# LeoQLi/DeepSIR

Hardware: AMD Instinct MI355X
Metric: registered pairs/sec (5k-pt 3DMatch-shaped synthetic pairs, 5 registration iterations, KNN pyramid included) (higher is better)
Workload: dtype f32 (GEMMs as fp16-pair MFMA, fp32 accumulate; index decisions exact fp32)

## Files before the change

### deepsir_amd/csrc/agg_chain_h.hip

```cpp
#include <hip/hip_fp16.h>

#include "kernels.h"
#include "device_utils.h"

namespace dsir {

namespace {

typedef _Float16 h8 __attribute__((ext_vector_type(8)));

constexpr int SRS = 80;
constexpr int LDT = 68;

__device__ __forceinline__ void split8(const float4 u, const float4 v, h8& h, h8& l) {
  const float f[8] = {u.x, u.y, u.z, u.w, v.x, v.y, v.z, v.w};
#pragma unroll
  for (int k = 0; k < 8; ++k) {
    const _Float16 t = (_Float16)f[k];
    h[k] = t;
    l[k] = (_Float16)(f[k] - (float)t);
  }
}

#define DSIR_MFMA16(acc, a, b) acc = __builtin_amdgcn_mfma_f32_16x16x32_f16(a, b, acc, 0, 0, 0)

template <int RT>
__global__ __launch_bounds__(256, 2) void agg_chain_h_kernel(const AggArgs p) {
  __shared__ _Float16 Bs[2][2][64 * SRS];
  __shared__ float Ts[4][RT][16 * LDT];

  const int tid = threadIdx.x, lane = tid & 63, w = __builtin_amdgcn_readfirstlane(tid >> 6);
  const int fr = lane & 15, fq = lane >> 4;
  const int cloud = blockIdx.y;
  const int r0 = blockIdx.x * (64 * RT) + 16 * RT * w;

  auto chunk_src = [&](int i, int& layer, int& ld, int& col0, int& k0, int& nk) {
    if (i == 0) { layer = 0; ld = 32; col0 = 0; k0 = 0; nk = 32; }
    else if (i <= 2) { layer = 1; ld = 64; col0 = 64 * (i - 1); k0 = 0; nk = 64; }
    else if (i == 15) { layer = 4; ld = 64; col0 = 0; k0 = 0; nk = 64; }
    else {
      const int j = (i - 3) / 3, u = (i - 3) % 3;
      if (u < 2) { layer = 2; ld = 128; col0 = 64 * j; k0 = 64 * u; nk = 64; }
      else { layer = 3; ld = 256; col0 = 0; k0 = 64 * j; nk = 64; }
    }
  };
  h8 rwh[2][2], rwl[2][2];
  auto gload = [&](int i) {
    int layer, ld, col0, k0, nk;
    chunk_src(i, layer, ld, col0, k0, nk);
    const _Float16* Wh = reinterpret_cast<const _Float16*>(p.Wh[layer]);
    const _Float16* Wl = reinterpret_cast<const _Float16*>(p.Wl[layer]);
#pragma unroll
    for (int u = 0; u < 2; ++u) {
      const int f = tid + 256 * u;
      const int piece = min(f & 7, nk / 8 - 1);
      const int64_t o = (int64_t)(col0 + (f >> 3)) * ld + k0 + 8 * piece;
      rwh[i & 1][u] = *reinterpret_cast<const h8*>(Wh + o);
      rwl[i & 1][u] = *reinterpret_cast<const h8*>(Wl + o);
    }
  };
  auto lstore = [&](int buf, int i) {
#pragma unroll
    for (int u = 0; u < 2; ++u) {
      const int f = tid + 256 * u;
      *reinterpret_cast<h8*>(&Bs[buf][0][(f >> 3) * SRS + 8 * (f & 7)]) = rwh[i & 1][u];
      *reinterpret_cast<h8*>(&Bs[buf][1][(f >> 3) * SRS + 8 * (f & 7)]) = rwl[i & 1][u];
    }
  };
  int buf = 0, ci = 0;
  auto next_chunk = [&]() {
    if (ci + 1 < 16) lstore(buf ^ 1, ci + 1);
    __syncthreads();
    buf ^= 1;
    ++ci;
    if (ci + 2 < 16) gload(ci + 2);
  };

  gload(0);
  lstore(0, 0);
  gload(1);
  gload(2);

  {
    float w1[2], b1[2];
#pragma unroll
    for (int t = 0; t < 2; ++t) { w1[t] = p.W1[(16 * t + fr) * 4 + fq]; b1[t] = p.b1[16 * t + fr]; }
#pragma unroll
    for (int rt = 0; rt < RT; ++rt) {
      const int row = min(r0 + 16 * rt + fr, p.n - 1);
      const float a = fq < 3 ? p.xyz[cloud * p.xyz_cs + (int64_t)row * 3 + fq] : p.score[(int64_t)cloud * p.n + row];
      float* T = Ts[w][rt];
#pragma unroll
      for (int t = 0; t < 2; ++t) {
        f32x4 c = __builtin_amdgcn_mfma_f32_16x16x4f32(a, w1[t], f32x4{0.f, 0.f, 0.f, 0.f}, 0, 0, 0);
#pragma unroll
        for (int r = 0; r < 4; ++r) {
          float v = c[r] + b1[t];
          v = v < 0.f ? v * 0.2f : v;
          T[(4 * fq + r) * LDT + 16 * t + fr] = v;
        }
      }
    }
  }
  __syncthreads();

  struct AFrag { h8 h[2], l[2]; };
  auto spill = [&](float* T, const f32x4 (&acc)[4], const float* bias, bool act) {
    __builtin_amdgcn_wave_barrier();
#pragma unroll
    for (int t = 0; t < 4; ++t) {
      const float b = bias[16 * t + fr];
#pragma unroll
      for (int r = 0; r < 4; ++r) {
        float v = acc[t][r] + b;
        if (act) v = v < 0.f ? v * 0.2f : v;
        T[(4 * fq + r) * LDT + 16 * t + fr] = v;
      }
    }
    __builtin_amdgcn_wave_barrier();
  };
  auto read_frag = [&](const float* T, AFrag& a, bool both) {
    const float4* q = reinterpret_cast<const float4*>(T + fr * LDT + 8 * fq);
    split8(q[0], q[1], a.h[0], a.l[0]);
    if (both) split8(q[8], q[9], a.h[1], a.l[1]);
  };
  auto zero = [&](f32x4 (&acc)[RT][4]) {
#pragma unroll
    for (int rt = 0; rt < RT; ++rt)
#pragma unroll
      for (int t = 0; t < 4; ++t) acc[rt][t] = f32x4{0.f, 0.f, 0.f, 0.f};
  };
  auto mma = [&](f32x4 (&acc)[RT][4], const AFrag (&a)[RT], const int KS) {
    const _Float16* bh = &Bs[buf][0][fr * SRS + 8 * fq];
    const _Float16* bl = &Bs[buf][1][fr * SRS + 8 * fq];
#pragma unroll
    for (int t = 0; t < 4; ++t) {
#pragma unroll
      for (int s = 0; s < 2; ++s) {
        if (s < KS) {
          const h8 vh = *reinterpret_cast<const h8*>(bh + 16 * t * SRS + 32 * s);
          const h8 vl = *reinterpret_cast<const h8*>(bl + 16 * t * SRS + 32 * s);
#pragma unroll
          for (int rt = 0; rt < RT; ++rt) {
            DSIR_MFMA16(acc[rt][t], a[rt].l[s], vh);
            DSIR_MFMA16(acc[rt][t], a[rt].h[s], vl);
            DSIR_MFMA16(acc[rt][t], a[rt].h[s], vh);
          }
        }
      }
    }
  };

  AFrag a3[RT];
  {
    AFrag a2[RT];
#pragma unroll
    for (int rt = 0; rt < RT; ++rt) read_frag(Ts[w][rt], a2[rt], false);
    f32x4 acc[RT][4];
    zero(acc);
    mma(acc, a2, 1);
#pragma unroll
    for (int rt = 0; rt < RT; ++rt) {
      spill(Ts[w][rt], acc[rt], p.b2, true);
      read_frag(Ts[w][rt], a3[rt], true);
    }
    next_chunk();
  }

  AFrag a4[2][RT];
#pragma unroll
  for (int c = 0; c < 2; ++c) {
    f32x4 acc[RT][4];
    zero(acc);
    mma(acc, a3, 2);
#pragma unroll
    for (int rt = 0; rt < RT; ++rt) {
      spill(Ts[w][rt], acc[rt], p.b3 + 64 * c, true);
      read_frag(Ts[w][rt], a4[c][rt], true);
    }
    next_chunk();
  }

  f32x4 acc5[RT][4];
  zero(acc5);
  float fpre[RT][4][4];
#pragma unroll
  for (int j = 0; j < 4; ++j) {
    f32x4 acc[RT][4];
    zero(acc);
    if (j == 3) {
#pragma unroll
      for (int rt = 0; rt < RT; ++rt)
#pragma unroll
        for (int r = 0; r < 4; ++r) {
          const int row = min(r0 + 16 * rt + 4 * fq + r, p.n - 1);
          const float* f = p.F + ((int64_t)cloud * p.n + row) * 64 + fr;
#pragma unroll
          for (int t = 0; t < 4; ++t) fpre[rt][r][t] = f[16 * t];
        }
    }
    mma(acc, a4[0], 2);
    next_chunk();
    mma(acc, a4[1], 2);
    AFrag a5[RT];
#pragma unroll
    for (int rt = 0; rt < RT; ++rt) {
      spill(Ts[w][rt], acc[rt], p.b4 + 64 * j, true);
      read_frag(Ts[w][rt], a5[rt], true);
    }
    next_chunk();
    mma(acc5, a5, 2);
    next_chunk();
  }

  {
    AFrag a6[RT];
#pragma unroll
    for (int rt = 0; rt < RT; ++rt) {
      float* T = Ts[w][rt];
      __builtin_amdgcn_wave_barrier();
#pragma unroll
      for (int r = 0; r < 4; ++r) {
#pragma unroll
        for (int t = 0; t < 4; ++t) T[(4 * fq + r) * LDT + 16 * t + fr] = (acc5[rt][t][r] + p.b5[16 * t + fr]) + fpre[rt][r][t];
      }
      __builtin_amdgcn_wave_barrier();
      read_frag(T, a6[rt], true);
    }
    f32x4 acc[RT][4];
    zero(acc);
    mma(acc, a6, 2);
    float bv[4];
#pragma unroll
    for (int t = 0; t < 4; ++t) bv[t] = p.b6[16 * t + fr];
    float* Y = p.desc + (int64_t)cloud * p.n * 64;
#pragma unroll
    for (int rt = 0; rt < RT; ++rt) {
      float ss[4] = {0.f, 0.f, 0.f, 0.f};
      float v[4][4];
#pragma unroll
      for (int t = 0; t < 4; ++t)
#pragma unroll
        for (int r = 0; r < 4; ++r) {
          v[t][r] = acc[rt][t][r] + bv[t];
          ss[r] += v[t][r] * v[t][r];
        }
      const bool extras = p.sq || p.hi || p.packed_init;
      float* T = Ts[w][rt];
      if (extras) __builtin_amdgcn_wave_barrier();
#pragma unroll
      for (int r = 0; r < 4; ++r) {
        ss[r] += __shfl_xor(ss[r], 1); ss[r] += __shfl_xor(ss[r], 2);
        ss[r] += __shfl_xor(ss[r], 4); ss[r] += __shfl_xor(ss[r], 8);
        const float den = fmaxf(__fsqrt_rn(ss[r]), 1e-12f);
        const int row = r0 + 16 * rt + 4 * fq + r;
        if (extras) {
#pragma unroll
          for (int t = 0; t < 4; ++t) T[(4 * fq + r) * LDT + 16 * t + fr] = v[t][r] / den;
        } else if (row < p.n) {
#pragma unroll
          for (int t = 0; t < 4; ++t) Y[(int64_t)row * 64 + 16 * t + fr] = v[t][r] / den;
        }
      }
      if (extras) {
        __builtin_amdgcn_wave_barrier();
#pragma unroll
        for (int q = 0; q < 4; ++q) {
          const int lr = 4 * q + fq, row = r0 + 16 * rt + lr;
          const float4 d4 = *reinterpret_cast<const float4*>(T + lr * LDT + 4 * fr);
          const float s2 = sqnorm_row16(d4);
          if (row < p.n) {
            const int64_t gr = (int64_t)cloud * p.n + row;
            *reinterpret_cast<float4*>(Y + (int64_t)row * 64 + 4 * fr) = d4;
            if (p.hi) {
              dsir_h4 hh, ll;
              screen_split4(d4, hh, ll, nullptr);
              *reinterpret_cast<dsir_h4*>(reinterpret_cast<_Float16*>(p.hi) + gr * 64 + 4 * fr) = hh;
              *reinterpret_cast<dsir_h4*>(reinterpret_cast<_Float16*>(p.lo) + gr * 64 + 4 * fr) = ll;
            }
            if (fr == 0) {
              if (p.sq) p.sq[gr] = s2;
              if (p.packed_init) p.packed_init[gr] = ~0ull;
            }
          }
        }
      }
    }
  }
}

}

#define DSIR_SPLIT_LOOP                                 \
  for (size_t i = 0; i < n; ++i) {                      \
    const _Float16 t = (_Float16)w[i];                  \
    const _Float16 l = (_Float16)(w[i] - (float)t);     \
    __builtin_memcpy(hi + i, &t, 2);                    \
    __builtin_memcpy(lo + i, &l, 2);                    \
  }
#if !defined(__HIP_DEVICE_COMPILE__) && defined(__x86_64__)
__attribute__((target("f16c"))) static void split_weights_f16c(const float* w, size_t n, uint16_t* hi, uint16_t* lo) { DSIR_SPLIT_LOOP }
#endif
void split_weights_f16(const float* w, size_t n, uint16_t* hi, uint16_t* lo) {
#if !defined(__HIP_DEVICE_COMPILE__) && defined(__x86_64__)
  if (__builtin_cpu_supports("f16c")) { split_weights_f16c(w, n, hi, lo); return; }
#endif
  DSIR_SPLIT_LOOP
}
#undef DSIR_SPLIT_LOOP

bool launch_agg_chain_h(const AggArgs& a, hipStream_t st) {
  if (a.n <= 0 || a.clouds <= 0) return true;
  for (int l = 0; l < 5; ++l)
    if (!a.Wh[l] || !a.Wl[l]) return false;
  if ((int64_t)((a.n + 127) / 128) * a.clouds >= 256) {
    dim3 grid((a.n + 127) / 128, a.clouds);
    hipLaunchKernelGGL(agg_chain_h_kernel<2>, grid, dim3(256), 0, st, a);
  } else {
    dim3 grid((a.n + 63) / 64, a.clouds);
    hipLaunchKernelGGL(agg_chain_h_kernel<1>, grid, dim3(256), 0, st, a);
  }
  return true;
}

}
```

Before: 5112.

## Keep MLP chain activations in registers via transposed MFMA operand order

Swaps MFMA operand order so the weights become the A operand and activations the B operand. Each layer's output accumulator can then be repacked directly into the next layer's fp16 hi/lo fragment in registers, without spilling through LDS and reading back. To make this work, the weight LDS store layout is permuted and biases and residual features are loaded as float4 in the transposed orientation. The per-wave LDS tile shrinks to a single buffer used only for the final extras path. This removes LDS round-trips and wave barriers between layers but may raise register pressure.

Result: no change. 5135, median of 5 (+0.5%).

```diff
diff --git a/deepsir_amd/csrc/agg_chain_h.hip b/deepsir_amd/csrc/agg_chain_h.hip
--- a/deepsir_amd/csrc/agg_chain_h.hip
+++ b/deepsir_amd/csrc/agg_chain_h.hip
@@ -8,6 +8,7 @@
 namespace {
 
 typedef _Float16 h8 __attribute__((ext_vector_type(8)));
+typedef _Float16 h4 __attribute__((ext_vector_type(4)));
 
 constexpr int SRS = 80;
 constexpr int LDT = 68;
@@ -27,7 +28,7 @@
 template <int RT>
 __global__ __launch_bounds__(256, 2) void agg_chain_h_kernel(const AggArgs p) {
   __shared__ _Float16 Bs[2][2][64 * SRS];
-  __shared__ float Ts[4][RT][16 * LDT];
+  __shared__ float Ts[4][16 * LDT];
 
   const int tid = threadIdx.x, lane = tid & 63, w = __builtin_amdgcn_readfirstlane(tid >> 6);
   const int fr = lane & 15, fq = lane >> 4;
@@ -63,8 +64,13 @@
 #pragma unroll
     for (int u = 0; u < 2; ++u) {
       const int f = tid + 256 * u;
-      *reinterpret_cast<h8*>(&Bs[buf][0][(f >> 3) * SRS + 8 * (f & 7)]) = rwh[i & 1][u];
-      *reinterpret_cast<h8*>(&Bs[buf][1][(f >> 3) * SRS + 8 * (f & 7)]) = rwl[i & 1][u];
+      const int c = f & 3;
+      const int o = (f >> 3) * SRS + 32 * ((f >> 2) & 1) + 16 * (c & 1) + 4 * (c >> 1);
+      const h8 vh = rwh[i & 1][u], vl = rwl[i & 1][u];
+      *reinterpret_cast<h4*>(&Bs[buf][0][o]) = h4{vh[0], vh[1], vh[2], vh[3]};
+      *reinterpret_cast<h4*>(&Bs[buf][0][o + 8]) = h4{vh[4], vh[5], vh[6], vh[7]};
+      *reinterpret_cast<h4*>(&Bs[buf][1][o]) = h4{vl[0], vl[1], vl[2], vl[3]};
+      *reinterpret_cast<h4*>(&Bs[buf][1][o + 8]) = h4{vl[4], vl[5], vl[6], vl[7]};
     }
   };
   int buf = 0, ci = 0;
@@ -81,188 +87,193 @@
   gload(1);
   gload(2);
 
+  struct BFrag { h8 h[2], l[2]; };
+  auto ldbias = [&](const float* bias, float (&b)[4][4]) {
+#pragma unroll
+    for (int t = 0; t < 4; ++t) {
+      const float4 q = *reinterpret_cast<const float4*>(bias + 16 * t + 4 * fq);
+      b[t][0] = q.x; b[t][1] = q.y; b[t][2] = q.z; b[t][3] = q.w;
+    }
+  };
+  auto pack = [&](const float (&v)[4][4], BFrag& o) {
+#pragma unroll
+    for (int s = 0; s < 2; ++s)
+#pragma unroll
+      for (int e = 0; e < 8; ++e) {
+        const float x = v[2 * s + (e >> 2)][e & 3];
+        const _Float16 t = (_Float16)x;
+        o.h[s][e] = t;
+        o.l[s][e] = (_Float16)(x - (float)t);
+      }
+  };
+  auto act_pack = [&](const f32x4 (&acc)[4], const float (&b)[4][4], BFrag& o) {
+    float v[4][4];
+#pragma unroll
+    for (int t = 0; t < 4; ++t)
+#pragma unroll
+      for (int r = 0; r < 4; ++r) {
+        const float x = acc[t][r] + b[t][r];
+        v[t][r] = x < 0.f ? x * 0.2f : x;
+      }
+    pack(v, o);
+  };
+
+  BFrag a2[RT];
   {
-    float w1[2], b1[2];
-#pragma unroll
-    for (int t = 0; t < 2; ++t) { w1[t] = p.W1[(16 * t + fr) * 4 + fq]; b1[t] = p.b1[16 * t + fr]; }
+    float w1[2], b1[2][4];
+#pragma unroll
+    for (int t = 0; t < 2; ++t) {
+      w1[t] = p.W1[(16 * t + fr) * 4 + fq];
+      const float4 q = *reinterpret_cast<const float4*>(p.b1 + 16 * t + 4 * fq);
+      b1[t][0] = q.x; b1[t][1] = q.y; b1[t][2] = q.z; b1[t][3] = q.w;
+    }
 #pragma unroll
     for (int rt = 0; rt < RT; ++rt) {
       const int row = min(r0 + 16 * rt + fr, p.n - 1);
       const float a = fq < 3 ? p.xyz[cloud * p.xyz_cs + (int64_t)row * 3 + fq] : p.score[(int64_t)cloud * p.n + row];
-      float* T = Ts[w][rt];
 #pragma unroll
       for (int t = 0; t < 2; ++t) {
-        f32x4 c = __builtin_amdgcn_mfma_f32_16x16x4f32(a, w1[t], f32x4{0.f, 0.f, 0.f, 0.f}, 0, 0, 0);
+        f32x4 c = __builtin_amdgcn_mfma_f32_16x16x4f32(w1[t], a, f32x4{0.f, 0.f, 0.f, 0.f}, 0, 0, 0);
 #pragma unroll
         for (int r = 0; r < 4; ++r) {
-          float v = c[r] + b1[t];
+          float v = c[r] + b1[t][r];
           v = v < 0.f ? v * 0.2f : v;
-          T[(4 * fq + r) * LDT + 16 * t + fr] = v;
+          const _Float16 hh = (_Float16)v;
+          a2[rt].h[0][4 * t + r] = hh;
+          a2[rt].l[0][4 * t + r] = (_Float16)(v - (float)hh);
         }
       }
     }
   }
   __syncthreads();
 
-  struct AFrag { h8 h[2], l[2]; };
-  auto spill = [&](float* T, const f32x4 (&acc)[4], const float* bias, bool act) {
-    __builtin_amdgcn_wave_barrier();
-#pragma unroll
-    for (int t = 0; t < 4; ++t) {
-      const float b = bias[16 * t + fr];
-#pragma unroll
-      for (int r = 0; r < 4; ++r) {
-        float v = acc[t][r] + b;
-        if (act) v = v < 0.f ? v * 0.2f : v;
-        T[(4 * fq + r) * LDT + 16 * t + fr] = v;
-      }
-    }
-    __builtin_amdgcn_wave_barrier();
-  };
-  auto read_frag = [&](const float* T, AFrag& a, bool both) {
-    const float4* q = reinterpret_cast<const float4*>(T + fr * LDT + 8 * fq);
-    split8(q[0], q[1], a.h[0], a.l[0]);
-    if (both) split8(q[8], q[9], a.h[1], a.l[1]);
-  };
   auto zero = [&](f32x4 (&acc)[RT][4]) {
 #pragma unroll
     for (int rt = 0; rt < RT; ++rt)
 #pragma unroll
       for (int t = 0; t < 4; ++t) acc[rt][t] = f32x4{0.f, 0.f, 0.f, 0.f};
   };
-  auto mma = [&](f32x4 (&acc)[RT][4], const AFrag (&a)[RT], const int KS) {
-    const _Float16* bh = &Bs[buf][0][fr * SRS + 8 * fq];
-    const _Float16* bl = &Bs[buf][1][fr * SRS + 8 * fq];
+  auto mma = [&](f32x4 (&acc)[RT][4], const BFrag (&b)[RT], const int KS) {
+    const _Float16* wh = &Bs[buf][0][fr * SRS + 8 * fq];
+    const _Float16* wl = &Bs[buf][1][fr * SRS + 8 * fq];
 #pragma unroll
     for (int t = 0; t < 4; ++t) {
 #pragma unroll
       for (int s = 0; s < 2; ++s) {
         if (s < KS) {
-          const h8 vh = *reinterpret_cast<const h8*>(bh + 16 * t * SRS + 32 * s);
-          const h8 vl = *reinterpret_cast<const h8*>(bl + 16 * t * SRS + 32 * s);
+          const h8 vh = *reinterpret_cast<const h8*>(wh + 16 * t * SRS + 32 * s);
+          const h8 vl = *reinterpret_cast<const h8*>(wl + 16 * t * SRS + 32 * s);
 #pragma unroll
           for (int rt = 0; rt < RT; ++rt) {
-            DSIR_MFMA16(acc[rt][t], a[rt].l[s], vh);
-            DSIR_MFMA16(acc[rt][t], a[rt].h[s], vl);
-            DSIR_MFMA16(acc[rt][t], a[rt].h[s], vh);
+            DSIR_MFMA16(acc[rt][t], vh, b[rt].l[s]);
+            DSIR_MFMA16(acc[rt][t], vl, b[rt].h[s]);
+            DSIR_MFMA16(acc[rt][t], vh, b[rt].h[s]);
           }
         }
       }
     }
   };
 
-  AFrag a3[RT];
+  float bias[4][4];
+  BFrag a3[RT];
   {
-    AFrag a2[RT];
-#pragma unroll
-    for (int rt = 0; rt < RT; ++rt) read_frag(Ts[w][rt], a2[rt], false);
+    ldbias(p.b2, bias);
     f32x4 acc[RT][4];
     zero(acc);
     mma(acc, a2, 1);
 #pragma unroll
-    for (int rt = 0; rt < RT; ++rt) {
-      spill(Ts[w][rt], acc[rt], p.b2, true);
-      read_frag(Ts[w][rt], a3[rt], true);
-    }
-    next_chunk();
-  }
-
-  AFrag a4[2][RT];
+    for (int rt = 0; rt < RT; ++rt) act_pack(acc[rt], bias, a3[rt]);
+    next_chunk();
+  }
+
+  BFrag a4[2][RT];
 #pragma unroll
   for (int c = 0; c < 2; ++c) {
+    ldbias(p.b3 + 64 * c, bias);
     f32x4 acc[RT][4];
     zero(acc);
     mma(acc, a3, 2);
 #pragma unroll
-    for (int rt = 0; rt < RT; ++rt) {
-      spill(Ts[w][rt], acc[rt], p.b3 + 64 * c, true);
-      read_frag(Ts[w][rt], a4[c][rt], true);
-    }
+    for (int rt = 0; rt < RT; ++rt) act_pack(acc[rt], bias, a4[c][rt]);
     next_chunk();
   }
 
   f32x4 acc5[RT][4];
   zero(acc5);
-  float fpre[RT][4][4];
+  float4 fpre[RT][4];
 #pragma unroll
   for (int j = 0; j < 4; ++j) {
     f32x4 acc[RT][4];
     zero(acc);
+    ldbias(p.b4 + 64 * j, bias);
     if (j == 3) {
 #pragma unroll
-      for (int rt = 0; rt < RT; ++rt)
-#pragma unroll
-        for (int r = 0; r < 4; ++r) {
-          const int row = min(r0 + 16 * rt + 4 * fq + r, p.n - 1);
-          const float* f = p.F + ((int64_t)cloud * p.n + row) * 64 + fr;
-#pragma unroll
-          for (int t = 0; t < 4; ++t) fpre[rt][r][t] = f[16 * t];
-        }
+      for (int rt = 0; rt < RT; ++rt) {
+        const int row = min(r0 + 16 * rt + fr, p.n - 1);
+        const float* f = p.F + ((int64_t)cloud * p.n + row) * 64 + 4 * fq;
+#pragma unroll
+        for (int t = 0; t < 4; ++t) fpre[rt][t] = *reinterpret_cast<const float4*>(f + 16 * t);
+      }
     }
     mma(acc, a4[0], 2);
     next_chunk();
     mma(acc, a4[1], 2);
-    AFrag a5[RT];
+    BFrag a5[RT];
+#pragma unroll
+    for (int rt = 0; rt < RT; ++rt) act_pack(acc[rt], bias, a5[rt]);
+    next_chunk();
+    mma(acc5, a5, 2);
+    next_chunk();
+  }
+
+  {
+    BFrag a6[RT];
+    ldbias(p.b5, bias);
 #pragma unroll
     for (int rt = 0; rt < RT; ++rt) {
-      spill(Ts[w][rt], acc[rt], p.b4 + 64 * j, true);
-      read_frag(Ts[w][rt], a5[rt], true);
-    }
-    next_chunk();
-    mma(acc5, a5, 2);
-    next_chunk();
-  }
-
-  {
-    AFrag a6[RT];
-#pragma unroll
-    for (int rt = 0; rt < RT; ++rt) {
-      float* T = Ts[w][rt];
-      __builtin_amdgcn_wave_barrier();
-#pragma unroll
-      for (int r = 0; r < 4; ++r) {
-#pragma unroll
-        for (int t = 0; t < 4; ++t) T[(4 * fq + r) * LDT + 16 * t + fr] = (acc5[rt][t][r] + p.b5[16 * t + fr]) + fpre[rt][r][t];
-      }
-      __builtin_amdgcn_wave_barrier();
-      read_frag(T, a6[rt], true);
-    }
+      float v[4][4];
+#pragma unroll
+      for (int t = 0; t < 4; ++t) {
+        const float f[4] = {fpre[rt][t].x, fpre[rt][t].y, fpre[rt][t].z, fpre[rt][t].w};
+#pragma unroll
+        for (int r = 0; r < 4; ++r) v[t][r] = (acc5[rt][t][r] + bias[t][r]) + f[r];
+      }
+      pack(v, a6[rt]);
+    }
+    ldbias(p.b6, bias);
     f32x4 acc[RT][4];
     zero(acc);
     mma(acc, a6, 2);
-    float bv[4];
-#pragma unroll
-    for (int t = 0; t < 4; ++t) bv[t] = p.b6[16 * t + fr];
     float* Y = p.desc + (int64_t)cloud * p.n * 64;
+    const bool extras = p.sq || p.hi || p.packed_init;
+    float* T = Ts[w];
 #pragma unroll
     for (int rt = 0; rt < RT; ++rt) {
-      float ss[4] = {0.f, 0.f, 0.f, 0.f};
       float v[4][4];
+      float ss = 0.f;
 #pragma unroll
       for (int t = 0; t < 4; ++t)
 #pragma unroll
         for (int r = 0; r < 4; ++r) {
-          v[t][r] = acc[rt][t][r] + bv[t];
-          ss[r] += v[t][r] * v[t][r];
-        }
-      const bool extras = p.sq || p.hi || p.packed_init;
-      float* T = Ts[w][rt];
-      if (extras) __builtin_amdgcn_wave_barrier();
-#pragma unroll
-      for (int r = 0; r < 4; ++r) {
-        ss[r] += __shfl_xor(ss[r], 1); ss[r] += __shfl_xor(ss[r], 2);
-        ss[r] += __shfl_xor(ss[r], 4); ss[r] += __shfl_xor(ss[r], 8);
-        const float den = fmaxf(__fsqrt_rn(ss[r]), 1e-12f);
-        const int row = r0 + 16 * rt + 4 * fq + r;
-        if (extras) {
-#pragma unroll
-          for (int t = 0; t < 4; ++t) T[(4 * fq + r) * LDT + 16 * t + fr] = v[t][r] / den;
-        } else if (row < p.n) {
-#pragma unroll
-          for (int t = 0; t < 4; ++t) Y[(int64_t)row * 64 + 16 * t + fr] = v[t][r] / den;
-        }
-      }
-      if (extras) {
+          v[t][r] = acc[rt][t][r] + bias[t][r];
+          ss += v[t][r] * v[t][r];
+        }
+      ss += __shfl_xor(ss, 16);
+      ss += __shfl_xor(ss, 32);
+      const float den = fmaxf(__fsqrt_rn(ss), 1e-12f);
+      const int prow = r0 + 16 * rt + fr;
+      if (!extras) {
+        if (prow < p.n) {
+#pragma unroll
+          for (int t = 0; t < 4; ++t)
+            *reinterpret_cast<float4*>(Y + (int64_t)prow * 64 + 16 * t + 4 * fq) =
+                make_float4(v[t][0] / den, v[t][1] / den, v[t][2] / den, v[t][3] / den);
+        }
+      } else {
+        __builtin_amdgcn_wave_barrier();
+#pragma unroll
+        for (int t = 0; t < 4; ++t)
+          *reinterpret_cast<float4*>(T + fr * LDT + 16 * t + 4 * fq) = make_float4(v[t][0] / den, v[t][1] / den, v[t][2] / den, v[t][3] / den);
         __builtin_amdgcn_wave_barrier();
 #pragma unroll
         for (int q = 0; q < 4; ++q) {
```
